# shg8/3DGS.cpp

Measured on NVIDIA H100. Metric: frames/sec, higher is better.
Workload: dtype f32

## Files before the change

3dgs.cpp_b200/csrc/gsb_api.cu:

```cuda
#include <float.h>
#include <math.h>
#include <stdio.h>
#include <stdlib.h>
#include <string.h>

#include <algorithm>
#include <new>
#include <thread>
#include <vector>

#include "gsb_ctx.cuh"

using namespace gsb;

namespace {
thread_local std::string g_create_error;
}

namespace gsb {

int fail(gsb_ctx* c, int code, const char* what, cudaError_t e) {
    if (c) {
        c->err = what;
        if (e != cudaSuccess) {
// ... 280 lines not shown
    }
    *out = fp;
    return GSB_OK;
}

ProjectParams project_params(const gsb_ctx* ctx, const gsb_uniforms& ubo, uint32_t rb, uint32_t re) {
    ProjectParams pp{};
    pp.pos_op = ctx->pos_op;
    pp.cov_a = ctx->cov_a;
    pp.cov_b = ctx->cov_b;
    pp.sh = ctx->sh;
    pp.sh_half = ctx->scene_sh_half ? 1 : 0;
    pp.n = (uint32_t)ctx->n;
    pp.ubo = ubo;
    pp.tile_row_begin = rb;
    pp.tile_row_end = re;
    pp.recs = ctx->recs;
    pp.dkeys = ctx->dkeys[0];
    pp.dvals = ctx->dvals[0];
    pp.status = ctx->project_status;
    pp.ctl = ctx->ctl;
    pp.dbg_tiles = ctx->dbg_tiles;
    pp.dbg_aabb = ctx->dbg_aabb;
    return pp;
}

static int enqueue_front(gsb_ctx* ctx, const gsb_uniforms* ubo, uint32_t rb, uint32_t re, const Survivors& sv, cudaStream_t stream,
                         FramePlan* out) {
    FramePlan fp{};
    int rc = plan_frame(ctx, ubo, rb, re, stream, &fp);
    if (rc != GSB_OK) return rc;
    const uint32_t chunks = (uint32_t)((ctx->n + 255) / 256);
    const bool timers = ctx->timers;
    CK(launch_frame_init(ctx->ctl, ctx->project_status, std::max(chunks, 1u), ctx->emit_status, std::max(chunks, 1u), ctx->ranges, fp.T, stream));
    if (timers) CK(cudaEventRecord(ctx->ev[0], stream));

    const bool fisheye = ctx->camera.kind == GSB_CAMERA_FISHEYE;
    CK(launch_project(project_params(ctx, *ubo, rb, re), ctx->debug, ctx->antialiased, stream, fisheye ? &ctx->camera : nullptr));
    if (timers) CK(cudaEventRecord(ctx->ev[1], stream));

    if (ctx->use_graph && !timers && !ctx->debug) rc = launch_middle_graph(ctx, fp, sv, stream);
    else rc = enqueue_middle(ctx, fp, sv, stream, timers);
    if (rc != GSB_OK) return rc;
    *out = fp;
    return GSB_OK;
}

int enqueue_blend(gsb_ctx* ctx, const FramePlan& fp, const Survivors& sv, uint32_t b0, uint32_t b1, void* band_out, size_t pitch,
                  int fmt, cudaStream_t stream, void* const* peer_frames, int num_peer_frames, void* depth_out, size_t depth_pitch) {
    BlendParams bp{};
    bp.recs = sv.recs;
    bp.vals = ctx->vals[fp.fin];
    bp.keys = ctx->keys[fp.fin];
    bp.ranges = ctx->ranges;
    bp.width = fp.W;
    bp.height = fp.H;
    bp.tiles_x = fp.tiles_x;
    bp.coarse_shift = fp.cs;
    bp.bins_x = fp.bins_x;
    bp.tile_row_begin = b0;
    bp.tile_row_end = b1;
    bp.out = static_cast<unsigned char*>(band_out) + (size_t)(b0 - fp.rb) * GSB_TILE * pitch;
    bp.out_first_row = b0 * GSB_TILE;
    bp.num_peers = num_peer_frames;
    for (int k = 0; k < num_peer_frames && k < GSB_MAX_SHARDS; k++) bp.peer_frames[k] = peer_frames[k];
    if (num_peer_frames > 0) bp.out_first_row = 0;
    bp.row_pitch_bytes = pitch;
// ... 148 lines not shown
    if (ctx->ctl) cudaFree(ctx->ctl);
    if (ctx->ctl_host) cudaFreeHost(ctx->ctl_host);
    for (auto& ev : ctx->ev)
        if (ev) cudaEventDestroy(ev);
    for (auto& ev : ctx->ev_sort)
        if (ev) cudaEventDestroy(ev);
    if (ctx->ev_done) cudaEventDestroy(ctx->ev_done);
    if (ctx->stream) cudaStreamDestroy(ctx->stream);
    delete ctx;
}

int gsb_scene_upload(gsb_ctx* ctx, const float* vertices, uint64_t n, gsb_memory mem) {
    if (!ctx) return GSB_ERR_INVALID;
    if (n && !vertices) return fail(ctx, GSB_ERR_INVALID, "null vertices");
    if (n >= (1ull << 30)) return fail(ctx, GSB_ERR_INVALID, "scene limited to 2^30 - 1 Gaussians");
    CK(cudaSetDevice(ctx->device));
    CK(cudaStreamSynchronize(ctx->stream));
    if (ctx->pos_op) CK(cudaDeviceSynchronize());
    ctx->frame.pending = ctx->frame.exists = false;
    ctx->n = 0;
    ctx->alloc_gen++;
    ctx->scene_gen++;
    drop_graphs(ctx);
    CK(ctx->pos_op.grow(n));
    CK(ctx->cov_a.grow(n));
    CK(ctx->cov_b.grow(n));
    ctx->scene_sh_half = ctx->sh_half;
    CK(ctx->sh.grow(n * (ctx->scene_sh_half ? 24 : 48)));
    CK(ctx->recs.grow(n * GSB_REC_F4));
    CK(ctx->dkeys[0].grow(n));
    CK(ctx->dkeys[1].grow(n));
    CK(ctx->dvals[0].grow(n));
    CK(ctx->dvals[1].grow(n));
    CK(ctx->project_status.grow((n + 255) / 256));
    CK(ctx->emit_status.grow((n + 255) / 256));
    if (ctx->debug) {
        CK(ctx->dbg_tiles.grow(n));
        CK(ctx->dbg_aabb.grow(n));
        CK(ctx->dbg_offsets.grow(n));
    }
    if (mem == GSB_MEM_DEVICE) {
        const uint64_t chunk = std::min<uint64_t>(std::max<uint64_t>(n, 1), 1u << 20);
        for (uint64_t off = 0; off < n; off += chunk) {
            const uint64_t cnt = std::min(chunk, n - off);
            cudaError_t e = launch_cov3d(vertices + off * 60, cnt, off, ctx->pos_op, ctx->cov_a, ctx->cov_b, ctx->sh, 1.0f, ctx->stream, ctx->scene_sh_half);
            if (e != cudaSuccess) return fail(ctx, GSB_ERR_CUDA, "cov3d precompute", e);
        }
        CK(cudaStreamSynchronize(ctx->stream));
    } else if (n) {
        cudaPointerAttributes pa{};
        const bool caller_pinned = cudaPointerGetAttributes(&pa, vertices) == cudaSuccess && pa.type == cudaMemoryTypeHost;
        cudaGetLastError();
        const uint64_t chunk = std::min<uint64_t>(n, 1u << 18);
        float* dev_stage[2] = {nullptr, nullptr};
        float* pin_stage[2] = {nullptr, nullptr};
        cudaEvent_t slot_free[2] = {nullptr, nullptr};
        cudaError_t e = cudaSuccess;
        for (int k = 0; k < 2 && e == cudaSuccess; k++) {
            e = dev_alloc(&dev_stage[k], chunk * 60);
            if (e == cudaSuccess && !caller_pinned) e = cudaMallocHost(reinterpret_cast<void**>(&pin_stage[k]), chunk * 60 * sizeof(float));
            if (e == cudaSuccess) e = cudaEventCreateWithFlags(&slot_free[k], cudaEventDisableTiming);
        }
        const unsigned hw = std::max(1u, std::min(std::thread::hardware_concurrency(), 8u));
        uint64_t idx = 0;
        for (uint64_t off = 0; off < n && e == cudaSuccess; off += chunk, idx++) {
            const int k = (int)(idx & 1);
            const uint64_t cnt = std::min(chunk, n - off);
// ... 976 lines not shown
```

3dgs.cpp_b200/csrc/gsb_internal.cuh:

```cuda
#pragma once
#include <cuda_runtime.h>
#include <stdint.h>

#include <string>

#include "gs_b200.h"

#define GSB_TILE 16
#define GSB_REC_F4 4
#define GSB_MAX_SHARDS 8

namespace gsb {

struct SortCtl {
    uint32_t ticket[8];
    uint32_t hist[8][256];
};

struct Control {
    uint32_t project_ticket;
    uint32_t emit_ticket;
    uint32_t num_visible;
    uint32_t num_instances;
    uint32_t overflow;
// ... 23 lines not shown
    uint32_t tile_row_begin, tile_row_end;
    float4* recs;
    uint32_t* dkeys;
    uint32_t* dvals;
    uint32_t* status;
    Control* ctl;
    uint32_t* dbg_tiles;
    uint4* dbg_aabb;
    int route_world;
    uint32_t band_rows;
    uint32_t* route_status;
    float4* route_dst_recs[GSB_MAX_SHARDS];
    uint32_t* route_dst_dkeys[GSB_MAX_SHARDS];
};

struct EmitParams {
    const uint32_t* sorted_cid;
    uint32_t nv_hint;
    uint32_t tiles_x;
    uint32_t* keys;
    uint32_t* vals;
    uint32_t capacity;
    unsigned long long* status;
    Control* ctl;
    int num_sms;
    const float4* recs;
    int cull;
    uint32_t coarse_shift;
    unsigned long long* dbg_offsets;
};

cudaError_t launch_cov3d(const float* vtx_aos, uint64_t count, uint64_t dst_offset, float4* pos_op,
                         float4* cov_a, float2* cov_b, float* sh, float scale_factor, cudaStream_t s, bool sh_half = false);
cudaError_t launch_project(const ProjectParams& p, bool debug, bool antialiased, cudaStream_t s, const gsb_camera_model* fisheye = nullptr);
cudaError_t launch_emit(const EmitParams& p, cudaStream_t s);

struct SortParams {
    void* keys[2] = {};
    uint32_t* vals[2] = {};
    int key_bytes = 4;
    const uint32_t* d_m = nullptr;
    uint32_t m_hint = 0;
    uint32_t key_bits = 0;
    unsigned long long* status = nullptr;
    uint32_t status_tiles = 0;
    const uint32_t* d_epoch = nullptr;
    uint32_t epoch_base = 0;
    SortCtl* sc = nullptr;
    int num_sms = 0;
    cudaEvent_t* events = nullptr;
    uint2* ranges = nullptr;
    uint32_t range_key_mask = 0;
    bool discard_sorted_keys = false;
};
cudaError_t launch_sort(const SortParams& p, uint32_t* passes, cudaStream_t s);
uint32_t sort_tile_items();

cudaError_t launch_frame_init(Control* ctl, uint32_t* project_status, uint32_t project_chunks, unsigned long long* emit_status,
                              uint32_t emit_chunks, uint2* ranges, uint32_t num_tiles, cudaStream_t s, uint32_t* route_status = nullptr,
                              uint32_t route_words = 0);
cudaError_t sort_prepare();
cudaError_t launch_ranges_single_tile(const uint32_t* d_m, uint2* ranges, cudaStream_t s);

struct BlendParams {
    const float4* recs;
    const uint32_t* vals;
// ... 136 lines not shown
```

3dgs.cpp_b200/csrc/gsb_preprocess.cu:

```cuda
#include <cuda_fp16.h>

#include <type_traits>

#include "gsb_cull.cuh"
#include "gsb_geom.cuh"
#include "gsb_internal.cuh"

namespace gsb {

namespace {

constexpr int PRE_THREADS = 256;
constexpr unsigned FULL = 0xffffffffu;

template <typename T>
__device__ __forceinline__ T ld_vol(const T* p) {
    return *reinterpret_cast<const volatile T*>(p);
}
template <typename T>
__device__ __forceinline__ void st_vol(T* p, T v) {
    *reinterpret_cast<volatile T*>(p) = v;
}

template <typename W>
// ... 82 lines not shown
}

template <bool SH16>
__device__ __forceinline__ void compute_sh(const float4* __restrict__ sh4, float px, float py, float pz,
                                           const float* cam, float& r, float& g, float& b) {
    ShDir d;
    view_direction(cam, px, py, pz, d.x, d.y, d.z);
    const float xx = d.x * d.x, yy = d.y * d.y;
    d.w6 = ((2.0f * d.z) * d.z - xx) - yy;
    d.w8 = xx - yy;
    d.w9 = (3.0f * d.x) * d.x - yy;
    d.w11 = ((4.0f * d.z) * d.z - xx) - yy;
    d.w12 = ((2.0f * d.z) * d.z - (3.0f * d.x) * d.x) - (3.0f * d.y) * d.y;
    d.w15 = xx - (3.0f * d.y) * d.y;
    float c[3] = {0.f, 0.f, 0.f};
    sh_group<0, SH16>(sh4, c, d);
    sh_group<1, SH16>(sh4, c, d);
    sh_group<2, SH16>(sh4, c, d);
    sh_group<3, SH16>(sh4, c, d);
    c[0] = c[0] + 0.5f;
    c[1] = c[1] + 0.5f;
    c[2] = c[2] + 0.5f;
    r = c[0] < 0.0f ? 0.0f : c[0];
    g = c[1];
    b = c[2];
}

#ifndef GSB_PROJECT_MIN_BLOCKS
#define GSB_PROJECT_MIN_BLOCKS 6
#endif
#ifndef GSB_PROJECT_FISHEYE_MIN_BLOCKS
#define GSB_PROJECT_FISHEYE_MIN_BLOCKS 4
#endif
struct ProjectFisheyeParams : ProjectParams {
    gsb_camera_model cam;
};
template <bool FISHEYE>
using ProjParams = std::conditional_t<FISHEYE, ProjectFisheyeParams, ProjectParams>;
template <bool FISHEYE>
struct ProjectBounds {
    static constexpr int MIN_BLOCKS = GSB_PROJECT_MIN_BLOCKS;
};
template <>
struct ProjectBounds<true> {
    static constexpr int MIN_BLOCKS = GSB_PROJECT_FISHEYE_MIN_BLOCKS;
};
template <bool DEBUG, bool ROUTED, bool SH16, bool AA, bool FISHEYE = false>
__global__ void __launch_bounds__(PRE_THREADS, ProjectBounds<FISHEYE>::MIN_BLOCKS) k_project(const __grid_constant__ ProjParams<FISHEYE> P) {
    static_assert(!(ROUTED && AA), "sharded contexts have no anti-aliased mode");
    static_assert(!(ROUTED && FISHEYE), "sharded contexts have no fisheye camera");
    __shared__ uint32_t s_chunk;
    __shared__ uint32_t s_wsurv[PRE_THREADS / 32];
    __shared__ uint32_t s_base_surv;
    __shared__ uint32_t s_rcnt[ROUTED ? PRE_THREADS / 32 : 1][GSB_MAX_SHARDS];
    __shared__ uint32_t s_rbase[GSB_MAX_SHARDS];

    const int tid = threadIdx.x, lane = tid & 31, warp = tid >> 5;
    if (tid == 0) s_chunk = atomicAdd(&P.ctl->project_ticket, 1u);
    __syncthreads();
    const uint32_t chunk = s_chunk;
    const uint32_t num_chunks = (P.n + PRE_THREADS - 1) / PRE_THREADS;
    const uint32_t i = chunk * PRE_THREADS + tid;

    const gsb_uniforms& U = P.ubo;
    const int W = (int)U.width, H = (int)U.height;
    const int tiles_x = (int)((U.width + GSB_TILE - 1) / GSB_TILE);
    const int tiles_y = (int)((U.height + GSB_TILE - 1) / GSB_TILE);

    bool surv = false;
    uint32_t nt = 0;
    float uvx = 0.f, uvy = 0.f, conx = 0.f, cony = 0.f, conz = 0.f, opac = 0.f, depth = 0.f, radii = 0.f;
    float px = 0.f, py = 0.f, pz = 0.f;
    int bx0 = 0, by0 = 0, bx1 = 0, by1 = 0;

    if (i < P.n) {
        const float4 po = __ldg(P.pos_op + i);
        px = po.x;
        py = po.y;
        pz = po.z;
        opac = po.w;
        const ClipView cv = clip_view(U, px, py, pz);
        const float ndcx = cv.ndcx, ndcy = cv.ndcy, vz = cv.vz;
        FisheyeGeo F;
        bool front;
        if constexpr (FISHEYE) {
            F = fisheye_geo(P.cam, cv.vx, cv.vy, vz);
            front = F.d > 0.2f && F.theta <= P.cam.max_theta;
        } else {
            front = !(vz <= 0.2f);
        }
        if (front) {
            Cov2d cov;
            if constexpr (FISHEYE) {
                const FisheyeJ J = fisheye_jacobian(P.cam, U.view_mat, F, cv.vx, cv.vy);
                cov = cov2d(J.T0, J.T1, __ldg(P.cov_a + i), __ldg(P.cov_b + i));
            } else {
                const Jacobian J = jacobian(U, cv.vx, cv.vy, vz);
                cov = cov2d(J.T0, J.T1, __ldg(P.cov_a + i), __ldg(P.cov_b + i));
            }
            const float m00 = cov.m00, m01 = cov.m01, m10 = cov.m10, m11 = cov.m11;
            const float det = m00 * m11 - m10 * m01;
            if (!(det <= 0.0f)) {
                const float ood = 1.0f / det;
                conx = m11 * ood;
                cony = -m01 * ood;
                conz = m00 * ood;
                if constexpr (AA) opac = opac * aa_compensation(aa_det0(cov), det);
                const float mid = 0.5f * (m00 + m11);
                const float sq = sqrtf(fmaxf(0.1f, mid * mid - det));
                const float lambda = fmaxf(mid + sq, mid - sq);
                radii = ceilf(3.0f * sqrtf(lambda));
                if constexpr (FISHEYE) {
                    uvx = P.cam.fx * (F.s * cv.vx) + P.cam.cx;
                    uvy = P.cam.fy * (F.s * cv.vy) + P.cam.cy;
                } else {
                    uvx = ((ndcx + 1.0f) * (float)W - 1.0f) * 0.5f;
                    uvy = ((ndcy + 1.0f) * (float)H - 1.0f) * 0.5f;
                }
                bx0 = clampi(__float2int_rz((uvx - radii) / 16.0f), 0, tiles_x);
                by0 = clampi(__float2int_rz((uvy - radii) / 16.0f), 0, tiles_y);
                bx1 = clampi(__float2int_rz((((uvx + radii) + 16.0f) - 1.0f) / 16.0f), 0, tiles_x);
                by1 = clampi(__float2int_rz((((uvy + radii) + 16.0f) - 1.0f) / 16.0f), 0, tiles_y);
                if ((uint32_t)by0 < P.tile_row_begin) by0 = (int)P.tile_row_begin;
                if ((uint32_t)by1 > P.tile_row_end) by1 = (int)P.tile_row_end;
                if (by1 < by0) by1 = by0;
                nt = (uint32_t)(bx1 - bx0) * (uint32_t)(by1 - by0);
                surv = nt != 0;
                depth = FISHEYE ? F.d : vz;
            }
        }
    }

    if constexpr (ROUTED) {
        const int G = P.route_world;
        uint32_t touch = 0;
        unsigned long long ranks = 0ull;
#pragma unroll
        for (int d = 0; d < GSB_MAX_SHARDS; d++) {
            if (d < G) {
                const int b0 = d * (int)P.band_rows, b1 = b0 + (int)P.band_rows;
                const bool t = surv && max(by0, b0) < min(by1, b1);
                const unsigned bits = __ballot_sync(FULL, t);
                if (t) touch |= 1u << d;
                ranks |= (unsigned long long)__popc(bits & ((1u << lane) - 1u)) << (5 * d);
                if (lane == 0) s_rcnt[warp][d] = __popc(bits);
            }
        }
        __syncthreads();
        if (tid < G) {
            uint32_t run = 0;
#pragma unroll
            for (int w = 0; w < PRE_THREADS / 32; w++) {
                const uint32_t c = s_rcnt[w][tid];
                s_rcnt[w][tid] = run;
                run += c;
            }
            s_rbase[tid] = run;
            st_vol(P.route_status + (size_t)chunk * GSB_MAX_SHARDS + tid, Lookback<uint32_t>::aggregate(chunk, run));
        }
        float colr = 0.f, colg = 0.f, colb = 0.f;
        if (surv) compute_sh<SH16>(reinterpret_cast<const float4*>(P.sh) + (size_t)i * (SH16 ? 6 : 12), px, py, pz, U.camera_position, colr, colg, colb);
        __syncthreads();
        if (warp < G) {
            const int d = warp;
            const uint32_t total = s_rbase[d];
            const uint32_t ex = lookback_exclusive(P.route_status + d, GSB_MAX_SHARDS, chunk, lane, total);
            __syncwarp();
            if (lane == 0) {
                s_rbase[d] = ex;
                if (chunk == num_chunks - 1) P.ctl->route_total[d] = ex + total;
            }
        }
        __syncthreads();
        if (touch) {
            const float4 q0 = make_float4(uvx, uvy, conx, cony);
            const float4 q2 = make_float4(colr, colg, colb, depth);
            const float4 q3 = make_float4(radii, __uint_as_float(P.index_base + i), 0.f, 0.f);
            const uint32_t dk = __float_as_uint(depth);
#pragma unroll
            for (int d = 0; d < GSB_MAX_SHARDS; d++) {
                if (d < G && ((touch >> d) & 1u)) {
                    const uint32_t pos = s_rbase[d] + s_rcnt[warp][d] + (uint32_t)((ranks >> (5 * d)) & 31ull);
                    const int b0 = d * (int)P.band_rows, b1 = b0 + (int)P.band_rows;
                    const int cy0 = max(by0, b0), cy1 = min(by1, b1);
                    float4* dst = P.route_dst_recs[d] + (size_t)pos * GSB_REC_F4;
                    dst[0] = q0;
                    dst[1] = make_float4(conz, opac, __uint_as_float((uint32_t)bx0 | ((uint32_t)cy0 << 16)),
                                         __uint_as_float((uint32_t)(bx1 - bx0) | ((uint32_t)(cy1 - cy0) << 16)));
                    dst[2] = q2;
                    dst[3] = q3;
                    P.route_dst_dkeys[d][pos] = dk;
                }
            }
        }
    } else {
    const unsigned surv_mask = __ballot_sync(FULL, surv);
    const uint32_t surv_rank_w = __popc(surv_mask & ((1u << lane) - 1u));
    if (lane == 0) s_wsurv[warp] = __popc(surv_mask);
    __syncthreads();
    uint32_t surv_before = 0, blk_surv = 0;
#pragma unroll
    for (int w = 0; w < PRE_THREADS / 32; w++) {
        const uint32_t a = s_wsurv[w];
        if (w < warp) surv_before += a;
        blk_surv += a;
    }
    if (tid == 0) st_vol(P.status + chunk, Lookback<uint32_t>::aggregate(chunk, blk_surv));

    float colr = 0.f, colg = 0.f, colb = 0.f;
    if (surv) compute_sh<SH16>(reinterpret_cast<const float4*>(P.sh) + (size_t)i * (SH16 ? 6 : 12), px, py, pz, U.camera_position, colr, colg, colb);

    if (warp == 0) {
        const uint32_t ex = lookback_exclusive(P.status, 1u, chunk, lane, blk_surv);
        if (lane == 0) {
            s_base_surv = ex;
            if (chunk == num_chunks - 1) P.ctl->num_visible = ex + blk_surv;
        }
    }
    __syncthreads();

    if (surv) {
        const uint32_t cid = s_base_surv + surv_before + surv_rank_w;
        float4* rec = P.recs + (size_t)cid * GSB_REC_F4;
        rec[0] = make_float4(uvx, uvy, conx, cony);
        rec[1] = make_float4(conz, opac, __uint_as_float((uint32_t)bx0 | ((uint32_t)by0 << 16)),
                             __uint_as_float((uint32_t)(bx1 - bx0) | ((uint32_t)(by1 - by0) << 16)));
        rec[2] = make_float4(colr, colg, colb, depth);
        rec[3] = make_float4(radii, __uint_as_float(P.index_base + i), 0.f, 0.f);
        P.dkeys[cid] = __float_as_uint(depth);
        P.dvals[cid] = cid;
    }
    }
    if (DEBUG && i < P.n) {
        P.dbg_tiles[i] = nt;
        P.dbg_aabb[i] = surv ? make_uint4(bx0, by0, bx1, by1) : make_uint4(0, 0, 0, 0);
    }
}

#ifndef GSB_EMIT_WIN
#define GSB_EMIT_WIN 4096
#endif
#ifndef GSB_EMIT_MIN_BLOCKS
#define GSB_EMIT_MIN_BLOCKS 5
#endif
constexpr int EMIT_WIN = GSB_EMIT_WIN;
constexpr uint32_t EMIT_BIG = 128;

__device__ __forceinline__ void emit_store_total(const EmitParams& P, unsigned long long total) {
    P.ctl->instances_total = total;
    P.ctl->num_instances = total > P.capacity ? P.capacity : (uint32_t)total;
    P.ctl->overflow = total > P.capacity ? 1u : 0u;
    if (total > P.capacity) atomicOr(&P.ctl->overflow_sticky, 1u);
}

__device__ __forceinline__ void emit_copy_out(const EmitParams& P, const uint32_t* s_key, const uint32_t* s_val,
                                              unsigned long long first_slot, uint32_t n, int tid) {
    for (uint32_t i = tid; i < n; i += PRE_THREADS) {
        const unsigned long long slot = first_slot + i;
        if (slot < P.capacity) {
            P.keys[slot] = s_key[i];
            P.vals[slot] = s_val[i];
        }
    }
}

__device__ __forceinline__ uint32_t coarse_tile_mask(uint32_t cs, uint32_t bx, uint32_t by, uint32_t x0, uint32_t y0, uint32_t x1, uint32_t y1) {
    const uint32_t ox = bx << cs, oy = by << cs, n = 1u << cs;
    const uint32_t lx0 = max(x0, ox) - ox, lx1 = min(x1, ox + n) - ox, ly0 = max(y0, oy) - oy, ly1 = min(y1, oy + n) - oy;
// ... 349 lines not shown
                const unsigned long long ex = lookback_exclusive(P.status, 1u, chunk, lane, (unsigned long long)blk_nt);
                if (lane == 0) {
                    s_base = ex;
                    if (chunk == num_chunks - 1) emit_store_total(P, ex + blk_nt);
                }
            }
            __syncthreads();
            if (w0 == 0) base = s_base;
            emit_copy_out(P, s_key, s_val, base + w0, w1 - w0, tid);
            __syncthreads();
        }
    }
}

}

template <bool AA, bool FISHEYE>
void launch_project_plain(const ProjParams<FISHEYE>& p, bool debug, unsigned blocks, cudaStream_t s) {
    if (p.sh_half) {
        if (debug) k_project<true, false, true, AA, FISHEYE><<<blocks, PRE_THREADS, 0, s>>>(p);
        else k_project<false, false, true, AA, FISHEYE><<<blocks, PRE_THREADS, 0, s>>>(p);
    } else if (debug) k_project<true, false, false, AA, FISHEYE><<<blocks, PRE_THREADS, 0, s>>>(p);
    else k_project<false, false, false, AA, FISHEYE><<<blocks, PRE_THREADS, 0, s>>>(p);
}

template <bool FISHEYE>
void launch_project_plain(const ProjParams<FISHEYE>& p, bool debug, bool antialiased, unsigned blocks, cudaStream_t s) {
    if (antialiased) launch_project_plain<true, FISHEYE>(p, debug, blocks, s);
    else launch_project_plain<false, FISHEYE>(p, debug, blocks, s);
}

cudaError_t launch_project(const ProjectParams& p, bool debug, bool antialiased, cudaStream_t s, const gsb_camera_model* fisheye) {
    if (p.n == 0) return cudaSuccess;
    const unsigned blocks = (p.n + PRE_THREADS - 1) / PRE_THREADS;
    if (p.route_world > 0) {
        if (antialiased || fisheye) return cudaErrorInvalidValue;
        if (p.sh_half) k_project<false, true, true, false><<<blocks, PRE_THREADS, 0, s>>>(p);
        else k_project<false, true, false, false><<<blocks, PRE_THREADS, 0, s>>>(p);
    } else if (fisheye) {
        launch_project_plain<true>(ProjectFisheyeParams{p, *fisheye}, debug, antialiased, blocks, s);
    } else {
        launch_project_plain<false>(p, debug, antialiased, blocks, s);
    }
    return cudaGetLastError();
}

cudaError_t launch_emit(const EmitParams& p, cudaStream_t s) {
    uint32_t blocks = (p.nv_hint + PRE_THREADS - 1) / PRE_THREADS;
    const uint32_t cap = (uint32_t)p.num_sms * 8;
    if (blocks > cap) blocks = cap;
    if (blocks == 0) blocks = 1;
    if (p.cull) k_emit<true><<<blocks, PRE_THREADS, 0, s>>>(p);
    else if (p.coarse_shift) k_emit_coarse<<<std::max<uint32_t>(1u, std::min<uint32_t>((p.nv_hint + EC_CHUNK - 1) / EC_CHUNK, cap)), PRE_THREADS, 0, s>>>(p);
    else k_emit<false><<<blocks, PRE_THREADS, 0, s>>>(p);
    return cudaGetLastError();
}

}
```

3dgs.cpp_b200/csrc/gsb_shard.cu:

```cuda
#include <dlfcn.h>
#include <nccl.h>
#include <stdio.h>
#include <stdlib.h>
#include <string.h>

#include <new>
#include <vector>

#include "gsb_ctx.cuh"

using namespace gsb;

namespace gsb {

struct Mailbox {
    uint32_t reserved[GSB_MAX_SHARDS];
    uint32_t routed[GSB_MAX_SHARDS];
    uint32_t framed[GSB_MAX_SHARDS];
    uint32_t count[2][GSB_MAX_SHARDS];
    uint32_t overflow[2][GSB_MAX_SHARDS];
    uint32_t error;
    uint32_t pad[7];
};
static_assert(sizeof(Mailbox) == 256, "mailbox layout");
// ... 248 lines not shown
    return w;
}

constexpr long long WAIT_TIMEOUT_CYCLES = 6000000000ll;

struct ShardFrame {
    gsb_uniforms ubo;
    int fmt = 0;
    cudaStream_t stream = nullptr;
    uint32_t f = 0, R = 0, tiles_y = 0, rb = 0, re = 0;
    int par = 0;
    FramePlan fp{};
};

int enqueue_sharded_phase(gsb_ctx* ctx, ShardFrame& F, int phase) {
    ShardState* sh = ctx->shard;
    const int G = sh->world, r = sh->rank;
    cudaStream_t stream = F.stream;
    Mailbox* mb = sh->mailbox(r);
    if (phase == 1) {
        const gsb_uniforms* ubo = &F.ubo;
        const uint32_t H = ubo->height;
        F.tiles_y = (H + GSB_TILE - 1) / GSB_TILE;
        F.R = (F.tiles_y + G - 1) / G;
        F.rb = std::min(F.tiles_y, (uint32_t)r * F.R);
        F.re = std::min(F.tiles_y, F.rb + F.R);
        F.f = ++sh->frame;
        F.par = (int)(F.f & 1u);
        sh->last_parity = (uint32_t)F.par;
        const uint64_t n_local = ctx->n;
        int rc = plan_frame(ctx, ubo, F.rb, F.re, stream, &F.fp);
        if (rc != GSB_OK) return rc;
        F.fp.nv_q = std::min<uint32_t>(quantise_hint(ctx->nv_hint ? ctx->nv_hint : sh->cap), quantise_hint(sh->cap));
        const uint32_t chunks_local = (uint32_t)((n_local + 255) / 256), chunks_cap = (uint32_t)((sh->cap + 255) / 256);
        CK(launch_frame_init(ctx->ctl, ctx->project_status, std::max(chunks_local, 1u), sh->emit_status_d, std::max(chunks_cap, 1u), ctx->ranges,
                             F.fp.T, stream, sh->route_status, std::max(chunks_local, 1u) * GSB_MAX_SHARDS));
        if (ctx->timers) CK(cudaEventRecord(ctx->ev[0], stream));
        ProjectParams pp = project_params(ctx, F.ubo, 0, F.tiles_y);
        pp.index_base = (uint32_t)((uint64_t)r * sh->slice);
        pp.route_world = G;
        pp.band_rows = std::max(F.R, 1u);
        pp.route_status = sh->route_status;
        for (int d = 0; d < G; d++) {
            pp.route_dst_recs[d] = sh->recs_x(d, F.par) + (size_t)r * sh->slice * GSB_REC_F4;
            pp.route_dst_dkeys[d] = sh->dkeys_x(d, F.par) + (size_t)r * sh->slice;
        }
        CK(launch_project(pp, false, false, stream));
        k_shard_signal<<<1, 32, 0, stream>>>(words_of(sh, offsetof(Mailbox, routed), 1, 0), F.f, G,
                                             words_of(sh, offsetof(Mailbox, count), 1, F.par * GSB_MAX_SHARDS), ctx->ctl->route_total, 1);
        CK(cudaGetLastError());
        return GSB_OK;
    }
    if (phase == 2) {
        k_shard_wait<<<1, 32, 0, stream>>>(mb->routed, F.f, G, &mb->error, WAIT_TIMEOUT_CYCLES);
        if (ctx->timers) CK(cudaEventRecord(ctx->ev[1], stream));
        GatherParams gp{};
        gp.counts = mb->count[F.par];
        gp.dkeys_x = sh->dkeys_x(r, F.par);
        gp.slice = (uint32_t)sh->slice;
        gp.world = G;
        gp.dkeys = sh->dkeys_d[0];
        gp.dvals = sh->dvals_d[0];
        gp.ctl = ctx->ctl;
        k_shard_gather<<<std::min<uint32_t>((F.fp.nv_q + 255) / 256, (uint32_t)ctx->num_sms * 8u), 256, 0, stream>>>(gp);
        CK(cudaGetLastError());

        const Survivors sv{sh->recs_x(r, F.par), {sh->dkeys_d[0], sh->dkeys_d[1]}, {sh->dvals_d[0], sh->dvals_d[1]}, sh->emit_status_d};
// ... 61 lines not shown
    if (pitch == 0) pitch = tight;
    CK(cudaMemcpy2DAsync(out, pitch, sh->frame_x(sh->rank, (int)sh->last_parity), tight, tight, ubo->height,
                         out_mem == GSB_MEM_HOST ? cudaMemcpyDeviceToHost : cudaMemcpyDeviceToDevice, s));
    if (out_mem == GSB_MEM_HOST) CK(cudaStreamSynchronize(s));
    return GSB_OK;
}

int attach_shard(gsb_ctx* ctx, int rank, int world) {
    ShardState* sh = new (std::nothrow) ShardState();
    if (!sh) return GSB_ERR_OOM;
    sh->rank = rank;
    sh->world = world;
    if (const char* v = getenv("GSB_SHARD_GATHER")) sh->gather_nccl = strcmp(v, "nccl") == 0;
    ctx->shard = sh;
    CK(cudaMallocHost(reinterpret_cast<void**>(&sh->mailbox_host), sizeof(Mailbox)));
    memset(sh->mailbox_host, 0, sizeof(Mailbox));
    return GSB_OK;
}

int upload_slice(gsb_ctx* ctx, const float* vertices, uint64_t n_total, gsb_memory mem) {
    ShardState* sh = ctx->shard;
    if (n_total >= (1ull << 30)) return fail(ctx, GSB_ERR_INVALID, "scene limited to 2^30 - 1 Gaussians");
    sh->n_total = n_total;
    sh->slice = std::max<uint64_t>((n_total + sh->world - 1) / sh->world, 1);
    sh->cap = sh->slice * sh->world;
    const uint64_t first = std::min(n_total, (uint64_t)sh->rank * sh->slice), count = std::min(sh->slice, n_total - first);
    int rc = gsb_scene_upload(ctx, count ? vertices : nullptr, count, mem);
    if (rc != GSB_OK) return rc;
    CK(sh->dkeys_d[0].grow(sh->cap));
    CK(sh->dkeys_d[1].grow(sh->cap));
    CK(sh->dvals_d[0].grow(sh->cap));
    CK(sh->dvals_d[1].grow(sh->cap));
    CK(sh->emit_status_d.grow((sh->cap + 255) / 256));
    CK(sh->route_status.grow(((sh->slice + 255) / 256) * GSB_MAX_SHARDS));
    ctx->alloc_gen++;
    rc = ensure_sort_status(ctx, std::max<uint64_t>(sh->cap, ctx->capacity));
    if (rc != GSB_OK) return rc;
    if (ctx->capacity < sh->slice * 2) rc = ensure_arena(ctx, std::max<uint64_t>(sh->slice * 2, 1024));
    sh->frame_bytes = 0;
    sh->frame_w = sh->frame_h = 0;
    if (sh->window) cudaFree(sh->window);
    sh->window = nullptr;
    return rc;
}

int check_sharded_args(gsb_ctx* ctx, const gsb_uniforms* ubo, int fmt) {
    if (!ctx) return GSB_ERR_INVALID;
    if (!ctx->shard) return fail(ctx, GSB_ERR_INVALID, "not a sharded context (gsb_create_sharded / gsb_group_create)");
    if (!ubo) return fail(ctx, GSB_ERR_INVALID, "null argument");
    if (!ctx->shard->n_total || !ctx->pos_op) return fail(ctx, GSB_ERR_NO_SCENE, "no scene uploaded");
    const int rc = check_image(ctx, ubo, fmt);
    if (rc != GSB_OK) return rc;
    if (ctx->debug) return fail(ctx, GSB_ERR_INVALID, "gsb_set_debug is not available on a sharded context");
    return GSB_OK;
}

bool load_nccl(NcclApi* a, std::string* why) {
    const char* names[] = {"libnccl.so.2", "libnccl.so"};
    for (const char* nm : names) {
        a->lib = dlopen(nm, RTLD_NOW | RTLD_GLOBAL);
        if (a->lib) break;
    }
    if (!a->lib) {
        *why = std::string("libnccl.so.2 not found: ") + dlerror();
        return false;
    }
    a->GetUniqueId = reinterpret_cast<decltype(a->GetUniqueId)>(dlsym(a->lib, "ncclGetUniqueId"));
// ... 306 lines not shown
```

Baseline: 658.0.

## Stage projected records in shared memory and compact before SH and global writes

The projection kernel now stages each surviving Gaussian's record in shared memory and builds a compacted survivor list. The SH colour evaluation then runs only over compacted survivors, so warps are not idled by culled lanes, and the records are written to global memory with contiguous coalesced stores. A compile-time items-per-thread knob (default 1) lets one block process several Gaussians per chunk. The cost is 16 KB or more of static shared memory per block, which may reduce occupancy, plus extra __syncthreads barriers.

```diff
diff --git a/3dgs.cpp_b200/csrc/gsb_api.cu b/3dgs.cpp_b200/csrc/gsb_api.cu
--- a/3dgs.cpp_b200/csrc/gsb_api.cu
+++ b/3dgs.cpp_b200/csrc/gsb_api.cu
@@ -336,7 +336,8 @@
     if (rc != GSB_OK) return rc;
     const uint32_t chunks = (uint32_t)((ctx->n + 255) / 256);
     const bool timers = ctx->timers;
-    CK(launch_frame_init(ctx->ctl, ctx->project_status, std::max(chunks, 1u), ctx->emit_status, std::max(chunks, 1u), ctx->ranges, fp.T, stream));
+    CK(launch_frame_init(ctx->ctl, ctx->project_status, std::max(project_chunks(ctx->n), 1u), ctx->emit_status, std::max(chunks, 1u), ctx->ranges,
+                         fp.T, stream));
     if (timers) CK(cudaEventRecord(ctx->ev[0], stream));
 
     const bool fisheye = ctx->camera.kind == GSB_CAMERA_FISHEYE;
@@ -551,7 +552,7 @@
     CK(ctx->dkeys[1].grow(n));
     CK(ctx->dvals[0].grow(n));
     CK(ctx->dvals[1].grow(n));
-    CK(ctx->project_status.grow((n + 255) / 256));
+    CK(ctx->project_status.grow(project_chunks(n)));
     CK(ctx->emit_status.grow((n + 255) / 256));
     if (ctx->debug) {
         CK(ctx->dbg_tiles.grow(n));
diff --git a/3dgs.cpp_b200/csrc/gsb_internal.cuh b/3dgs.cpp_b200/csrc/gsb_internal.cuh
--- a/3dgs.cpp_b200/csrc/gsb_internal.cuh
+++ b/3dgs.cpp_b200/csrc/gsb_internal.cuh
@@ -79,6 +79,11 @@
 
 cudaError_t launch_cov3d(const float* vtx_aos, uint64_t count, uint64_t dst_offset, float4* pos_op,
                          float4* cov_a, float2* cov_b, float* sh, float scale_factor, cudaStream_t s, bool sh_half = false);
+#ifndef GSB_PROJECT_IPT
+#define GSB_PROJECT_IPT 1
+#endif
+constexpr uint32_t PROJECT_CHUNK = 256u * GSB_PROJECT_IPT;
+inline uint32_t project_chunks(uint64_t n) { return (uint32_t)((n + PROJECT_CHUNK - 1) / PROJECT_CHUNK); }
 cudaError_t launch_project(const ProjectParams& p, bool debug, bool antialiased, cudaStream_t s, const gsb_camera_model* fisheye = nullptr);
 cudaError_t launch_emit(const EmitParams& p, cudaStream_t s);
 
diff --git a/3dgs.cpp_b200/csrc/gsb_preprocess.cu b/3dgs.cpp_b200/csrc/gsb_preprocess.cu
--- a/3dgs.cpp_b200/csrc/gsb_preprocess.cu
+++ b/3dgs.cpp_b200/csrc/gsb_preprocess.cu
@@ -138,6 +138,9 @@
 #ifndef GSB_PROJECT_FISHEYE_MIN_BLOCKS
 #define GSB_PROJECT_FISHEYE_MIN_BLOCKS 4
 #endif
+constexpr int PROJ_IPT = GSB_PROJECT_IPT;
+static_assert((int)PROJECT_CHUNK == PRE_THREADS * PROJ_IPT, "k_project's chunk is PRE_THREADS x PROJ_IPT Gaussians");
+static_assert(PROJ_IPT == 1 || PROJ_IPT == 2, "k_project stages 64 B per chunk Gaussian in static shared memory (48 KB)");
 struct ProjectFisheyeParams : ProjectParams {
     gsb_camera_model cam;
 };
@@ -151,41 +154,27 @@
 struct ProjectBounds<true> {
     static constexpr int MIN_BLOCKS = GSB_PROJECT_FISHEYE_MIN_BLOCKS;
 };
-template <bool DEBUG, bool ROUTED, bool SH16, bool AA, bool FISHEYE = false>
-__global__ void __launch_bounds__(PRE_THREADS, ProjectBounds<FISHEYE>::MIN_BLOCKS) k_project(const __grid_constant__ ProjParams<FISHEYE> P) {
-    static_assert(!(ROUTED && AA), "sharded contexts have no anti-aliased mode");
-    static_assert(!(ROUTED && FISHEYE), "sharded contexts have no fisheye camera");
-    __shared__ uint32_t s_chunk;
-    __shared__ uint32_t s_wsurv[PRE_THREADS / 32];
-    __shared__ uint32_t s_base_surv;
-    __shared__ uint32_t s_rcnt[ROUTED ? PRE_THREADS / 32 : 1][GSB_MAX_SHARDS];
-    __shared__ uint32_t s_rbase[GSB_MAX_SHARDS];
-
-    const int tid = threadIdx.x, lane = tid & 31, warp = tid >> 5;
-    if (tid == 0) s_chunk = atomicAdd(&P.ctl->project_ticket, 1u);
-    __syncthreads();
-    const uint32_t chunk = s_chunk;
-    const uint32_t num_chunks = (P.n + PRE_THREADS - 1) / PRE_THREADS;
-    const uint32_t i = chunk * PRE_THREADS + tid;
-
+
+struct Projected {
+    bool surv;
+    uint32_t nt;
+    float uvx, uvy, conx, cony, conz, opac, depth, radii;
+    float px, py, pz;
+    int bx0, by0, bx1, by1;
+};
+
+template <bool AA, bool FISHEYE>
+__device__ __forceinline__ Projected project_one(const ProjParams<FISHEYE>& P, uint32_t i, int tiles_x, int tiles_y) {
     const gsb_uniforms& U = P.ubo;
     const int W = (int)U.width, H = (int)U.height;
-    const int tiles_x = (int)((U.width + GSB_TILE - 1) / GSB_TILE);
-    const int tiles_y = (int)((U.height + GSB_TILE - 1) / GSB_TILE);
-
-    bool surv = false;
-    uint32_t nt = 0;
-    float uvx = 0.f, uvy = 0.f, conx = 0.f, cony = 0.f, conz = 0.f, opac = 0.f, depth = 0.f, radii = 0.f;
-    float px = 0.f, py = 0.f, pz = 0.f;
-    int bx0 = 0, by0 = 0, bx1 = 0, by1 = 0;
-
+    Projected g{};
     if (i < P.n) {
         const float4 po = __ldg(P.pos_op + i);
-        px = po.x;
-        py = po.y;
-        pz = po.z;
-        opac = po.w;
-        const ClipView cv = clip_view(U, px, py, pz);
+        g.px = po.x;
+        g.py = po.y;
+        g.pz = po.z;
+        g.opac = po.w;
+        const ClipView cv = clip_view(U, g.px, g.py, g.pz);
         const float ndcx = cv.ndcx, ndcy = cv.ndcy, vz = cv.vz;
         FisheyeGeo F;
         bool front;
@@ -208,55 +197,121 @@
             const float det = m00 * m11 - m10 * m01;
             if (!(det <= 0.0f)) {
                 const float ood = 1.0f / det;
-                conx = m11 * ood;
-                cony = -m01 * ood;
-                conz = m00 * ood;
-                if constexpr (AA) opac = opac * aa_compensation(aa_det0(cov), det);
+                g.conx = m11 * ood;
+                g.cony = -m01 * ood;
+                g.conz = m00 * ood;
+                if constexpr (AA) g.opac = g.opac * aa_compensation(aa_det0(cov), det);
                 const float mid = 0.5f * (m00 + m11);
                 const float sq = sqrtf(fmaxf(0.1f, mid * mid - det));
                 const float lambda = fmaxf(mid + sq, mid - sq);
-                radii = ceilf(3.0f * sqrtf(lambda));
+                g.radii = ceilf(3.0f * sqrtf(lambda));
                 if constexpr (FISHEYE) {
-                    uvx = P.cam.fx * (F.s * cv.vx) + P.cam.cx;
-                    uvy = P.cam.fy * (F.s * cv.vy) + P.cam.cy;
+                    g.uvx = P.cam.fx * (F.s * cv.vx) + P.cam.cx;
+                    g.uvy = P.cam.fy * (F.s * cv.vy) + P.cam.cy;
                 } else {
-                    uvx = ((ndcx + 1.0f) * (float)W - 1.0f) * 0.5f;
-                    uvy = ((ndcy + 1.0f) * (float)H - 1.0f) * 0.5f;
-                }
-                bx0 = clampi(__float2int_rz((uvx - radii) / 16.0f), 0, tiles_x);
-                by0 = clampi(__float2int_rz((uvy - radii) / 16.0f), 0, tiles_y);
-                bx1 = clampi(__float2int_rz((((uvx + radii) + 16.0f) - 1.0f) / 16.0f), 0, tiles_x);
-                by1 = clampi(__float2int_rz((((uvy + radii) + 16.0f) - 1.0f) / 16.0f), 0, tiles_y);
-                if ((uint32_t)by0 < P.tile_row_begin) by0 = (int)P.tile_row_begin;
-                if ((uint32_t)by1 > P.tile_row_end) by1 = (int)P.tile_row_end;
-                if (by1 < by0) by1 = by0;
-                nt = (uint32_t)(bx1 - bx0) * (uint32_t)(by1 - by0);
-                surv = nt != 0;
-                depth = FISHEYE ? F.d : vz;
-            }
-        }
-    }
-
+                    g.uvx = ((ndcx + 1.0f) * (float)W - 1.0f) * 0.5f;
+                    g.uvy = ((ndcy + 1.0f) * (float)H - 1.0f) * 0.5f;
+                }
+                g.bx0 = clampi(__float2int_rz((g.uvx - g.radii) / 16.0f), 0, tiles_x);
+                g.by0 = clampi(__float2int_rz((g.uvy - g.radii) / 16.0f), 0, tiles_y);
+                g.bx1 = clampi(__float2int_rz((((g.uvx + g.radii) + 16.0f) - 1.0f) / 16.0f), 0, tiles_x);
+                g.by1 = clampi(__float2int_rz((((g.uvy + g.radii) + 16.0f) - 1.0f) / 16.0f), 0, tiles_y);
+                if ((uint32_t)g.by0 < P.tile_row_begin) g.by0 = (int)P.tile_row_begin;
+                if ((uint32_t)g.by1 > P.tile_row_end) g.by1 = (int)P.tile_row_end;
+                if (g.by1 < g.by0) g.by1 = g.by0;
+                g.nt = (uint32_t)(g.bx1 - g.bx0) * (uint32_t)(g.by1 - g.by0);
+                g.surv = g.nt != 0;
+                g.depth = FISHEYE ? F.d : vz;
+            }
+        }
+    }
+    return g;
+}
+
+template <bool DEBUG, bool ROUTED, bool SH16, bool AA, bool FISHEYE = false>
+__global__ void __launch_bounds__(PRE_THREADS, ProjectBounds<FISHEYE>::MIN_BLOCKS) k_project(const __grid_constant__ ProjParams<FISHEYE> P) {
+    static_assert(!(ROUTED && AA), "sharded contexts have no anti-aliased mode");
+    static_assert(!(ROUTED && FISHEYE), "sharded contexts have no fisheye camera");
+    constexpr int WARPS = PRE_THREADS / 32;
+    __shared__ uint32_t s_chunk;
+    __shared__ uint32_t s_wsurv[PROJ_IPT][WARPS];
+    __shared__ uint32_t s_base_surv;
+    __shared__ uint32_t s_rcnt[ROUTED ? PROJ_IPT * WARPS : 1][GSB_MAX_SHARDS];
+    __shared__ uint32_t s_rbase[GSB_MAX_SHARDS];
+    __shared__ float4 s_rec[PROJECT_CHUNK][GSB_REC_F4];
+    __shared__ uint16_t s_list[PROJECT_CHUNK];
+
+    const int tid = threadIdx.x, lane = tid & 31, warp = tid >> 5;
+    if (tid == 0) s_chunk = atomicAdd(&P.ctl->project_ticket, 1u);
+    __syncthreads();
+    const uint32_t chunk = s_chunk;
+    const uint32_t num_chunks = (P.n + PROJECT_CHUNK - 1) / PROJECT_CHUNK;
+    const uint32_t i0 = chunk * PROJECT_CHUNK;
+
+    const gsb_uniforms& U = P.ubo;
+    const int tiles_x = (int)((U.width + GSB_TILE - 1) / GSB_TILE);
+    const int tiles_y = (int)((U.height + GSB_TILE - 1) / GSB_TILE);
+
+    uint32_t rank[PROJ_IPT];
+    uint32_t touch[ROUTED ? PROJ_IPT : 1];
+    unsigned long long ranks[ROUTED ? PROJ_IPT : 1];
+    uint32_t survs = 0;
+#pragma unroll
+    for (int k = 0; k < PROJ_IPT; k++) {
+        const uint32_t pos = k * PRE_THREADS + tid, i = i0 + pos;
+        const Projected g = project_one<AA, FISHEYE>(P, i, tiles_x, tiles_y);
+        if (g.surv) {
+            survs |= 1u << k;
+            s_rec[pos][0] = make_float4(g.uvx, g.uvy, g.conx, g.cony);
+            s_rec[pos][1] = make_float4(g.conz, g.opac, __uint_as_float((uint32_t)g.bx0 | ((uint32_t)g.by0 << 16)),
+                                        __uint_as_float((uint32_t)(g.bx1 - g.bx0) | ((uint32_t)(g.by1 - g.by0) << 16)));
+            s_rec[pos][2] = make_float4(g.depth, g.px, g.py, g.pz);
+            s_rec[pos][3] = make_float4(g.radii, __uint_as_float(P.index_base + i), 0.f, 0.f);
+        }
+        const unsigned m = __ballot_sync(FULL, g.surv);
+        rank[k] = __popc(m & ((1u << lane) - 1u));
+        if (lane == 0) s_wsurv[k][warp] = __popc(m);
+        if constexpr (ROUTED) {
+            touch[k] = 0;
+            ranks[k] = 0ull;
+#pragma unroll
+            for (int d = 0; d < GSB_MAX_SHARDS; d++) {
+                if (d < P.route_world) {
+                    const int b0 = d * (int)P.band_rows, b1 = b0 + (int)P.band_rows;
+                    const bool t = g.surv && max(g.by0, b0) < min(g.by1, b1);
+                    const unsigned bits = __ballot_sync(FULL, t);
+                    if (t) touch[k] |= 1u << d;
+                    ranks[k] |= (unsigned long long)__popc(bits & ((1u << lane) - 1u)) << (5 * d);
+                    if (lane == 0) s_rcnt[k * WARPS + warp][d] = __popc(bits);
+                }
+            }
+        }
+        if (DEBUG && i < P.n) {
+            P.dbg_tiles[i] = g.nt;
+            P.dbg_aabb[i] = g.surv ? make_uint4(g.bx0, g.by0, g.bx1, g.by1) : make_uint4(0, 0, 0, 0);
+        }
+    }
+    __syncthreads();
+
+    uint32_t blk_surv = 0;
+#pragma unroll
+    for (int k = 0; k < PROJ_IPT; k++) {
+        uint32_t before = 0, tot = 0;
+#pragma unroll
+        for (int w = 0; w < WARPS; w++) {
+            const uint32_t a = s_wsurv[k][w];
+            if (w < warp) before += a;
+            tot += a;
+        }
+        rank[k] += blk_surv + before;
+        blk_surv += tot;
+        if ((survs >> k) & 1u) s_list[rank[k]] = (uint16_t)(k * PRE_THREADS + tid);
+    }
     if constexpr (ROUTED) {
-        const int G = P.route_world;
-        uint32_t touch = 0;
-        unsigned long long ranks = 0ull;
-#pragma unroll
-        for (int d = 0; d < GSB_MAX_SHARDS; d++) {
-            if (d < G) {
-                const int b0 = d * (int)P.band_rows, b1 = b0 + (int)P.band_rows;
-                const bool t = surv && max(by0, b0) < min(by1, b1);
-                const unsigned bits = __ballot_sync(FULL, t);
-                if (t) touch |= 1u << d;
-                ranks |= (unsigned long long)__popc(bits & ((1u << lane) - 1u)) << (5 * d);
-                if (lane == 0) s_rcnt[warp][d] = __popc(bits);
-            }
-        }
-        __syncthreads();
-        if (tid < G) {
+        if (tid < P.route_world) {
             uint32_t run = 0;
 #pragma unroll
-            for (int w = 0; w < PRE_THREADS / 32; w++) {
+            for (int w = 0; w < PROJ_IPT * WARPS; w++) {
                 const uint32_t c = s_rcnt[w][tid];
                 s_rcnt[w][tid] = run;
                 run += c;
@@ -264,10 +319,22 @@
             s_rbase[tid] = run;
             st_vol(P.route_status + (size_t)chunk * GSB_MAX_SHARDS + tid, Lookback<uint32_t>::aggregate(chunk, run));
         }
-        float colr = 0.f, colg = 0.f, colb = 0.f;
-        if (surv) compute_sh<SH16>(reinterpret_cast<const float4*>(P.sh) + (size_t)i * (SH16 ? 6 : 12), px, py, pz, U.camera_position, colr, colg, colb);
+    } else {
+        if (tid == 0) st_vol(P.status + chunk, Lookback<uint32_t>::aggregate(chunk, blk_surv));
+    }
+    __syncthreads();
+
+    for (uint32_t r = tid; r < blk_surv; r += PRE_THREADS) {
+        const uint32_t pos = s_list[r];
+        const float4 e = s_rec[pos][2];
+        float cr, cg, cb;
+        compute_sh<SH16>(reinterpret_cast<const float4*>(P.sh) + (size_t)(i0 + pos) * (SH16 ? 6 : 12), e.y, e.z, e.w, U.camera_position, cr, cg, cb);
+        s_rec[pos][2] = make_float4(cr, cg, cb, e.x);
+    }
+
+    if constexpr (ROUTED) {
         __syncthreads();
-        if (warp < G) {
+        if (warp < P.route_world) {
             const int d = warp;
             const uint32_t total = s_rbase[d];
             const uint32_t ex = lookback_exclusive(P.route_status + d, GSB_MAX_SHARDS, chunk, lane, total);
@@ -278,68 +345,46 @@
             }
         }
         __syncthreads();
-        if (touch) {
-            const float4 q0 = make_float4(uvx, uvy, conx, cony);
-            const float4 q2 = make_float4(colr, colg, colb, depth);
-            const float4 q3 = make_float4(radii, __uint_as_float(P.index_base + i), 0.f, 0.f);
-            const uint32_t dk = __float_as_uint(depth);
+#pragma unroll
+        for (int k = 0; k < PROJ_IPT; k++) {
+            if (!touch[k]) continue;
+            const uint32_t pos = k * PRE_THREADS + tid;
+            const float4 q0 = s_rec[pos][0], q1 = s_rec[pos][1], q2 = s_rec[pos][2], q3 = s_rec[pos][3];
+            const uint32_t xy = __float_as_uint(q1.z), wh = __float_as_uint(q1.w);
+            const int by0 = (int)(xy >> 16), by1 = by0 + (int)(wh >> 16);
+            const uint32_t dk = __float_as_uint(q2.w);
 #pragma unroll
             for (int d = 0; d < GSB_MAX_SHARDS; d++) {
-                if (d < G && ((touch >> d) & 1u)) {
-                    const uint32_t pos = s_rbase[d] + s_rcnt[warp][d] + (uint32_t)((ranks >> (5 * d)) & 31ull);
+                if (d < P.route_world && ((touch[k] >> d) & 1u)) {
+                    const uint32_t slot = s_rbase[d] + s_rcnt[k * WARPS + warp][d] + (uint32_t)((ranks[k] >> (5 * d)) & 31ull);
                     const int b0 = d * (int)P.band_rows, b1 = b0 + (int)P.band_rows;
                     const int cy0 = max(by0, b0), cy1 = min(by1, b1);
-                    float4* dst = P.route_dst_recs[d] + (size_t)pos * GSB_REC_F4;
+                    float4* dst = P.route_dst_recs[d] + (size_t)slot * GSB_REC_F4;
                     dst[0] = q0;
-                    dst[1] = make_float4(conz, opac, __uint_as_float((uint32_t)bx0 | ((uint32_t)cy0 << 16)),
-                                         __uint_as_float((uint32_t)(bx1 - bx0) | ((uint32_t)(cy1 - cy0) << 16)));
+                    dst[1] = make_float4(q1.x, q1.y, __uint_as_float((xy & 0xffffu) | ((uint32_t)cy0 << 16)),
+                                         __uint_as_float((wh & 0xffffu) | ((uint32_t)(cy1 - cy0) << 16)));
                     dst[2] = q2;
                     dst[3] = q3;
-                    P.route_dst_dkeys[d][pos] = dk;
+                    P.route_dst_dkeys[d][slot] = dk;
                 }
             }
         }
     } else {
-    const unsigned surv_mask = __ballot_sync(FULL, surv);
-    const uint32_t surv_rank_w = __popc(surv_mask & ((1u << lane) - 1u));
-    if (lane == 0) s_wsurv[warp] = __popc(surv_mask);
-    __syncthreads();
-    uint32_t surv_before = 0, blk_surv = 0;
-#pragma unroll
-    for (int w = 0; w < PRE_THREADS / 32; w++) {
-        const uint32_t a = s_wsurv[w];
-        if (w < warp) surv_before += a;
-        blk_surv += a;
-    }
-    if (tid == 0) st_vol(P.status + chunk, Lookback<uint32_t>::aggregate(chunk, blk_surv));
-
-    float colr = 0.f, colg = 0.f, colb = 0.f;
-    if (surv) compute_sh<SH16>(reinterpret_cast<const float4*>(P.sh) + (size_t)i * (SH16 ? 6 : 12), px, py, pz, U.camera_position, colr, colg, colb);
-
-    if (warp == 0) {
-        const uint32_t ex = lookback_exclusive(P.status, 1u, chunk, lane, blk_surv);
-        if (lane == 0) {
-            s_base_surv = ex;
-            if (chunk == num_chunks - 1) P.ctl->num_visible = ex + blk_surv;
-        }
-    }
-    __syncthreads();
-
-    if (surv) {
-        const uint32_t cid = s_base_surv + surv_before + surv_rank_w;
-        float4* rec = P.recs + (size_t)cid * GSB_REC_F4;
-        rec[0] = make_float4(uvx, uvy, conx, cony);
-        rec[1] = make_float4(conz, opac, __uint_as_float((uint32_t)bx0 | ((uint32_t)by0 << 16)),
-                             __uint_as_float((uint32_t)(bx1 - bx0) | ((uint32_t)(by1 - by0) << 16)));
-        rec[2] = make_float4(colr, colg, colb, depth);
-        rec[3] = make_float4(radii, __uint_as_float(P.index_base + i), 0.f, 0.f);
-        P.dkeys[cid] = __float_as_uint(depth);
-        P.dvals[cid] = cid;
-    }
-    }
-    if (DEBUG && i < P.n) {
-        P.dbg_tiles[i] = nt;
-        P.dbg_aabb[i] = surv ? make_uint4(bx0, by0, bx1, by1) : make_uint4(0, 0, 0, 0);
+        if (warp == 0) {
+            const uint32_t ex = lookback_exclusive(P.status, 1u, chunk, lane, blk_surv);
+            if (lane == 0) {
+                s_base_surv = ex;
+                if (chunk == num_chunks - 1) P.ctl->num_visible = ex + blk_surv;
+            }
+        }
+        __syncthreads();
+        const uint32_t base = s_base_surv;
+        float4* recs = P.recs + (size_t)base * GSB_REC_F4;
+        for (uint32_t f = tid; f < blk_surv * GSB_REC_F4; f += PRE_THREADS) recs[f] = s_rec[s_list[f / GSB_REC_F4]][f % GSB_REC_F4];
+        for (uint32_t r = tid; r < blk_surv; r += PRE_THREADS) {
+            P.dkeys[base + r] = __float_as_uint(s_rec[s_list[r]][2].w);
+            P.dvals[base + r] = base + r;
+        }
     }
 }
 
@@ -755,7 +800,7 @@
 
 cudaError_t launch_project(const ProjectParams& p, bool debug, bool antialiased, cudaStream_t s, const gsb_camera_model* fisheye) {
     if (p.n == 0) return cudaSuccess;
-    const unsigned blocks = (p.n + PRE_THREADS - 1) / PRE_THREADS;
+    const unsigned blocks = project_chunks(p.n);
     if (p.route_world > 0) {
         if (antialiased || fisheye) return cudaErrorInvalidValue;
         if (p.sh_half) k_project<false, true, true, false><<<blocks, PRE_THREADS, 0, s>>>(p);
diff --git a/3dgs.cpp_b200/csrc/gsb_shard.cu b/3dgs.cpp_b200/csrc/gsb_shard.cu
--- a/3dgs.cpp_b200/csrc/gsb_shard.cu
+++ b/3dgs.cpp_b200/csrc/gsb_shard.cu
@@ -304,7 +304,7 @@
         int rc = plan_frame(ctx, ubo, F.rb, F.re, stream, &F.fp);
         if (rc != GSB_OK) return rc;
         F.fp.nv_q = std::min<uint32_t>(quantise_hint(ctx->nv_hint ? ctx->nv_hint : sh->cap), quantise_hint(sh->cap));
-        const uint32_t chunks_local = (uint32_t)((n_local + 255) / 256), chunks_cap = (uint32_t)((sh->cap + 255) / 256);
+        const uint32_t chunks_local = project_chunks(n_local), chunks_cap = (uint32_t)((sh->cap + 255) / 256);
         CK(launch_frame_init(ctx->ctl, ctx->project_status, std::max(chunks_local, 1u), sh->emit_status_d, std::max(chunks_cap, 1u), ctx->ranges,
                              F.fp.T, stream, sh->route_status, std::max(chunks_local, 1u) * GSB_MAX_SHARDS));
         if (ctx->timers) CK(cudaEventRecord(ctx->ev[0], stream));
@@ -432,7 +432,7 @@
     CK(sh->dvals_d[0].grow(sh->cap));
     CK(sh->dvals_d[1].grow(sh->cap));
     CK(sh->emit_status_d.grow((sh->cap + 255) / 256));
-    CK(sh->route_status.grow(((sh->slice + 255) / 256) * GSB_MAX_SHARDS));
+    CK(sh->route_status.grow(project_chunks(sh->slice) * GSB_MAX_SHARDS));
     ctx->alloc_gen++;
     rc = ensure_sort_status(ctx, std::max<uint64_t>(sh->cap, ctx->capacity));
     if (rc != GSB_OK) return rc;
```

New measurement: 660.1, median of 6. About the same (+0.3%).
